# jkulhanek/viewformer

Measured on AMD Instinct MI355X. Metric: novel views/sec (encode->AR transformer->decode), 128px 6-ctx, higher is better.
Workload: dtype bf16

## Files before the change

__graft_entry__.py:

```python
import os
import sys

REPO = os.path.dirname(os.path.abspath(__file__))
if REPO not in sys.path:
    sys.path.insert(0, REPO)


def build() -> None:
    from viewformer_amd import build as vf_build
    lib = vf_build.build()
    assert os.path.exists(lib), lib
    var = vf_build.build_variant('trintrin')
    assert os.path.exists(var), var
    import viewformer_amd
    from viewformer_amd import _lib, vqgan, migt, evaluate
    _lib.load()
    import oracle.vqgan_oracle, oracle.migt_oracle, oracle.pipeline_oracle
    print('built', lib)


def smoke() -> None:
    import numpy as np
    import torch
    assert torch.cuda.is_available(), 'smoke() needs the MI355X'
    from viewformer_amd.config import VQGANConfig, MIGTConfig
    from viewformer_amd.weights import make_vqgan_weights, make_migt_weights, synthetic_scene_batch
    from viewformer_amd.vqgan import VQGAN
    from viewformer_amd.migt import MIGT
    from viewformer_amd.evaluate import generate_batch_predictions
    from oracle import pipeline_oracle as po

    dev = torch.device('cuda:0')
    vcfg = VQGANConfig(ch=32, ch_mult=[1, 2, 4], num_res_blocks=1, attn_resolutions=[16], image_size=32,
                       z_channels=32, embed_dim=32, n_embed=128)
    mcfg = MIGTConfig(n_embeddings=128, n_head=2, d_model=128, n_layer=2, token_image_size=8, sequence_size=3,
                      pose_multiplier=0.2)
    vsd = make_vqgan_weights(vcfg, seed=1, codebook_scale=0.05)
    msd = make_migt_weights(mcfg, seed=1, std=0.05)
    frames, cams = synthetic_scene_batch(2, 3, 32, seed=2)
    vq = VQGAN(vcfg, data_format='NHWC').load_state_dict(vsd).to(dev)
    tr = MIGT(mcfg).load_state_dict(msd).to(dev)
    got = generate_batch_predictions(tr, vq, frames, cams, return_codes=True)
    torch.cuda.synchronize()
    ref = po.generate_batch_predictions(msd, mcfg, vsd, vcfg, frames, cams, return_intermediates=True)
    assert torch.equal(got['codes'].cpu(), ref['codes']), 'context token indices differ from the oracle'
    err = (got['logits_last'].cpu() - ref['logits_last']).abs().max().item()
    assert err < 1e-3, err
    agree = (got['generated_codes'].cpu() == ref['generated_codes']).float().mean().item()
    assert agree > 0.95, agree
    print(f'smoke ok: context codes bit-exact, logit err {err:.2e}, generated-code agreement {agree:.3f}')


if __name__ == '__main__':
    build()
    if len(sys.argv) > 1 and sys.argv[1] == 'smoke':
        smoke()
```

viewformer_amd/build.py:

```python
import os
import subprocess
import sys

HERE = os.path.dirname(os.path.abspath(__file__))
CSRC = os.path.join(HERE, 'csrc')
LIB = os.path.join(HERE, 'libvf_hip.so')
ARCH = 'gfx950'
EXTRA_FLAGS = {'conv3_halo_x3h': ['-fno-slp-vectorize']}


def sources():
    return sorted(os.path.join(CSRC, f) for f in os.listdir(CSRC) if f.endswith('.hip'))


def _stale():
    if not os.path.exists(LIB):
        return True
    t = os.path.getmtime(LIB)
    deps = sources() + [os.path.join(CSRC, f) for f in os.listdir(CSRC) if f.endswith('.h')]
    deps.append(os.path.join(os.path.dirname(HERE), 'include', 'vf_hip.h'))
    return any(os.path.getmtime(d) > t for d in deps)


def build(force: bool = False, verbose: bool = False) -> str:
    if not force and not _stale():
        return LIB
    hipcc = os.environ.get('HIPCC', '/opt/rocm/bin/hipcc')
    objs = []
    procs = []
    os.makedirs(os.path.join(HERE, 'build'), exist_ok=True)
    stems = {os.path.basename(s)[:-4] for s in sources()}
    for f in os.listdir(os.path.join(HERE, 'build')):
        if f.endswith('.o') and f[:-2] not in stems:
            os.remove(os.path.join(HERE, 'build', f))
    for src in sources():
        obj = os.path.join(HERE, 'build', os.path.basename(src)[:-4] + '.o')
        cmd = [hipcc, f'--offload-arch={ARCH}', '-O3', '-std=c++17', '-fPIC', '-c', src, '-o', obj,
               '-Wall', '-Wno-unused-function'] + EXTRA_FLAGS.get(os.path.basename(src)[:-4], [])
        if verbose:
            cmd.append('-Rpass-analysis=kernel-resource-usage')
        procs.append((src, subprocess.Popen(cmd, stdout=subprocess.PIPE, stderr=subprocess.STDOUT, text=True)))
        objs.append(obj)
    failed = False
    for src, p in procs:
        out, _ = p.communicate()
        if p.returncode != 0 or verbose:
            sys.stderr.write(f'--- {os.path.basename(src)}\n{out}\n')
        failed |= p.returncode != 0
    if failed:
        raise RuntimeError('hipcc failed')
    cmd = [hipcc, f'--offload-arch={ARCH}', '-shared', '-fPIC', '-o', LIB] + objs
    subprocess.check_call(cmd)
    return LIB


VARIANTS = {
    'trintrin': (['-DVF_X_TRINTRIN'], ['attention_dma', 'attention_train_bf16', 'gemm_tn_bf16']),
}


def variant_path(name: str) -> str:
    return os.path.join(HERE, 'variants', f'libvf_{name}.so')


def build_variant(name: str, force: bool = False) -> str:
    flags, stems = VARIANTS[name]
    build()
    out = variant_path(name)
    srcs = [os.path.join(CSRC, st + '.hip') for st in stems]
    hdrs = [os.path.join(CSRC, f) for f in os.listdir(CSRC) if f.endswith('.h')]
    if not force and os.path.exists(out) and all(os.path.getmtime(d) <= os.path.getmtime(out) for d in srcs + hdrs + [LIB]):
        return out
    hipcc = os.environ.get('HIPCC', '/opt/rocm/bin/hipcc')
    os.makedirs(os.path.dirname(out), exist_ok=True)
    procs, vobjs = [], []
    for st, src in zip(stems, srcs):
        obj = os.path.join(HERE, 'variants', f'{st}.{name}.o')
        cmd = [hipcc, f'--offload-arch={ARCH}', '-O3', '-std=c++17', '-fPIC', '-w', '-c', src, '-o', obj] + EXTRA_FLAGS.get(st, []) + flags
        procs.append(subprocess.Popen(cmd))
        vobjs.append(obj)
    if any(p.wait() != 0 for p in procs):
        raise RuntimeError(f'hipcc failed on variant {name}')
    objs = [os.path.join(HERE, 'build', os.path.basename(s)[:-4] + '.o') for s in sources() if os.path.basename(s)[:-4] not in stems]
    subprocess.check_call([hipcc, f'--offload-arch={ARCH}', '-shared', '-fPIC', '-o', out] + objs + vobjs)
    return out


if __name__ == '__main__':
    print(build(force='--force' in sys.argv, verbose='-v' in sys.argv))
```

viewformer_amd/csrc/conv3_halo_bf16.hip:

```cpp
#include "halo_common.h"

namespace {

typedef __bf16 bf16x8 __attribute__((ext_vector_type(8)));
typedef __bf16 bf16x4 __attribute__((ext_vector_type(4)));

constexpr int CK = 32;
constexpr int P_LDB = 80;
constexpr int TH = 8, TW = 16;
constexpr int BN = 128;
constexpr int TAP_BYTES = CK * BN * 2;

template <bool UP2, bool PAIR = false>
struct Geo {
    static constexpr int PH = UP2 ? (TH / 2 + 2) : (TH + 2);
    static constexpr int PW = PAIR ? 20 : (UP2 ? (TW / 2 + 2) : (TW + 2));
    static constexpr int NPIX = PH * PW;
    static constexpr int SLOTS = (NPIX * 8 + 255) / 256;
    static constexpr int BUF = (NPIX + 1) * P_LDB;
};

__device__ __forceinline__ float fast_swish(float t) {
    return t * __builtin_amdgcn_rcpf(1.0f + __builtin_amdgcn_exp2f(-1.4426950408889634f * t));
}
// ... 95 lines not shown
    if (PAIR) { img = bid * 2; }
    else { tx = bid % tilesX; bid /= tilesX; ty = bid % tilesY; img = bid / tilesY; }
    const int n_img_total = p.M / (p.Hout * p.Wout);
    const int img1 = PAIR ? min(img + 1, n_img_total - 1) : img;
    const int pair_pix = (img1 - img) * p.Hin * p.Win;
    const int y0 = ty * TH, x0 = tx * TW;
    const int sy0 = UP2 ? (y0 / 2 - 1) : (y0 - 1);
    const int sx0 = UP2 ? (x0 / 2 - 1) : (x0 - 1);

    const float* __restrict__ X = p.x + (size_t)img * p.Hin * p.Win * p.Cin;
    const int nchunks = p.Cin / CK;
    const int last_stage = nchunks * 9 - 1;

    const int c4 = tid & 7;
    int s_off[G::SLOTS];
    bool s_ok[G::SLOTS];
    int s_sel[G::SLOTS];
    int s_lds[G::SLOTS];
#pragma unroll
    for (int q = 0; q < G::SLOTS; ++q) {
        const int pix = (tid >> 3) + 32 * q;
        const int pixc = pix < G::NPIX ? pix : G::NPIX;
        const int pr = pixc / G::PW, pc0 = pixc - pr * G::PW;
        const int sel = PAIR ? (pc0 >= 10) : 0;
        const int pc = pc0 - 10 * sel;
        s_sel[q] = sel;
        const int sy = sy0 + pr, sx = sx0 + pc;
        const bool ok = pix < G::NPIX && sy >= 0 && sy < p.Hin && sx >= 0 && sx < p.Win;
        s_ok[q] = ok;
        s_off[q] = ok ? (sel * pair_pix + sy * p.Win + sx) * p.Cin + c4 * 4 : c4 * 4;
        s_lds[q] = pixc * P_LDB + c4 * 8;
    }

    f32x4 preg[G::SLOTS];
    f32x4 pa, pb, pa1, pb1;
    const __amdgpu_buffer_rsrc_t x_rs = __builtin_amdgcn_make_buffer_rsrc(const_cast<float*>(X), 0, 0x7fffffff, 0x00020000);
    auto patch_load = [&](int chunk) {
#pragma unroll
        for (int q = 0; q < G::SLOTS; ++q)
            preg[q] = __builtin_bit_cast(f32x4, __builtin_amdgcn_raw_buffer_load_b128(x_rs, (unsigned)s_off[q] * 4u, (unsigned)(chunk * CK * 4), 0));
        if (PRO) {
            const f32x4 pmean = *reinterpret_cast<const f32x4*>(p.pro_mean + (size_t)img * p.Cin + chunk * CK + c4 * 4);
            const f32x4 pbeta = *reinterpret_cast<const f32x4*>(p.pro_beta + chunk * CK + c4 * 4);
            pa = *reinterpret_cast<const f32x4*>(p.pro_scale + (size_t)img * p.Cin + chunk * CK + c4 * 4);
#pragma unroll
            for (int e = 0; e < 4; ++e) pb[e] = __builtin_fmaf(-pmean[e], pa[e], pbeta[e]);
            if (PAIR) {
                const f32x4 pmean1 = *reinterpret_cast<const f32x4*>(p.pro_mean + (size_t)img1 * p.Cin + chunk * CK + c4 * 4);
                pa1 = *reinterpret_cast<const f32x4*>(p.pro_scale + (size_t)img1 * p.Cin + chunk * CK + c4 * 4);
#pragma unroll
                for (int e = 0; e < 4; ++e) pb1[e] = __builtin_fmaf(-pmean1[e], pa1[e], pbeta[e]);
            }
        }
    };
    auto patch_store_slot = [&](int buf, int q) {
        unsigned char* dst = smem_h + buf * G::BUF;
        bf16x4 o;
#pragma unroll
        for (int e = 0; e < 4; ++e) {
            float t = preg[q][e];
            if (PRO) {
                t = __builtin_fmaf(t, (PAIR && s_sel[q]) ? pa1[e] : pa[e], (PAIR && s_sel[q]) ? pb1[e] : pb[e]);
                if (SWISH) t = fast_swish(t);
            }
            o[e] = (__bf16)(s_ok[q] ? t : 0.f);
        }
        *reinterpret_cast<bf16x4*>(dst + s_lds[q]) = o;
    };

    const int trow = vf_perm_row(l31), tpx = vf_perm_px(l31);
    int a_base[MI], a_r[MI];
#pragma unroll
    for (int mi = 0; mi < MI; ++mi) {
        const int a0 = wave_m * 4 + mi * 2 + trow;
        a_r[mi] = a0;
        const int tcol = PAIR ? (tpx >> 3) * 10 + (tpx & 7) : tpx;
        a_base[mi] = (a0 * G::PW + tcol) * P_LDB + half * 16;
    }

    const unsigned char* __restrict__ Wb = reinterpret_cast<const unsigned char*>(p.w_packed) + (size_t)nblk * TAP_BYTES;
    const size_t tap_stride = (size_t)nb * TAP_BYTES;
    const int b_lane = (half * BN + wave_n * (32 * NJ) + l31) * 16;
    constexpr int BD = 2, RING = BD + 1;
    static_assert(9 % RING == 0, "ring indices must repeat per chunk");
    bf16x8 bring[RING][2 * NJ];
    bf16x8 aring[2][MI][2];
    const int last_g = nchunks * 9 - 1;
    const __amdgpu_buffer_rsrc_t w_rs = __builtin_amdgcn_make_buffer_rsrc(const_cast<unsigned char*>(Wb), 0, 0x7fffffff, 0x00020000);
    auto b_load = [&](bf16x8 (&dst)[2 * NJ], int g) {
        const unsigned soff = (unsigned)((size_t)min(g, last_g) * tap_stride);
#pragma unroll
        for (int ks = 0; ks < 2; ++ks)
#pragma unroll
            for (int j = 0; j < NJ; ++j)
                dst[ks * NJ + j] = __builtin_bit_cast(bf16x8, __builtin_amdgcn_raw_buffer_load_b128(w_rs, (unsigned)((ks * 2 * BN + j * 32) * 16 + b_lane), soff, 0));
    };
    auto a_load = [&](bf16x8 (&dst)[MI][2], const unsigned char* patch, int tap) {
        const int dy = tap / 3, dx = tap % 3;
#pragma unroll
        for (int mi = 0; mi < MI; ++mi) {
            int aoff;
            if (UP2) {
                const int pr = (a_r[mi] + dy + 1) >> 1, pc = (tpx + dx + 1) >> 1;
                aoff = (pr * G::PW + pc) * P_LDB + half * 16;
            } else {
                aoff = a_base[mi] + (dy * G::PW + dx) * P_LDB;
            }
#pragma unroll
            for (int ks = 0; ks < 2; ++ks) dst[mi][ks] = *reinterpret_cast<const bf16x8*>(patch + aoff + ks * 32);
        }
    };

    f32x16 acc[MI][NJ];
#pragma unroll
    for (int i = 0; i < MI; ++i)
#pragma unroll
        for (int j = 0; j < NJ; ++j)
#pragma unroll
            for (int r = 0; r < 16; ++r) acc[i][j][r] = 0.f;

    patch_load(0);
#pragma unroll
    for (int g = 0; g < BD; ++g) b_load(bring[g], g);
#pragma unroll
    for (int q = 0; q < G::SLOTS; ++q) patch_store_slot(0, q);
    __syncthreads();

    for (int chunk = 0; chunk < nchunks; ++chunk) {
        const unsigned char* patch = smem_h + (chunk & 1) * G::BUF;
        patch_load(min(chunk + 1, nchunks - 1));
        a_load(aring[0], patch, 0);
#pragma unroll
        for (int tap = 0; tap < 9; ++tap) {
            b_load(bring[(tap + BD) % RING], chunk * 9 + tap + BD);
            if (tap + 1 < 9) a_load(aring[(tap + 1) & 1], patch, tap + 1);
#pragma unroll
            for (int ks = 0; ks < 2; ++ks)
#pragma unroll
                for (int mi = 0; mi < MI; ++mi)
#pragma unroll
                    for (int j = 0; j < NJ; ++j)
                        acc[mi][j] = __builtin_amdgcn_mfma_f32_32x32x16_bf16(aring[tap & 1][mi][ks], bring[tap % RING][ks * NJ + j], acc[mi][j], 0, 0, 0);
            __builtin_amdgcn_sched_barrier(0);
            if (tap >= 1 && tap <= G::SLOTS) patch_store_slot((chunk + 1) & 1, tap - 1);
        }
        __syncthreads();
    }

    if constexpr (OUT16) halo_epilogue16<MI, NJ>(p, acc, img, y0, x0, (ty * tilesX + tx) * 2, nblk, wave_m, wave_n, half, l31);
    else vf_halo_epilogue_t<PAIR, MI, NJ>(p, acc, img, img1, y0, x0, PAIR ? 0 : (ty * tilesX + tx) * 2, nblk, wave_m, wave_n, half, l31);
}


template <bool UP2, bool PRO, bool SWISH>
__global__ __launch_bounds__(128, 2) void conv3_halo_bf16_w2_kernel(vf_igemm_args p) {
    using G = Geo<UP2, false>;
    constexpr int SLOTS = (G::NPIX + 31) / 32;
    constexpr int MI = 4, NJ = 2;
    extern __shared__ __attribute__((aligned(16))) unsigned char smem_h[];
    typedef unsigned u32x4 __attribute__((ext_vector_type(4)));

    const int tid = threadIdx.x;
    const int lane = tid & 63;
    const int wave_n = __builtin_amdgcn_readfirstlane(tid >> 6);
    const int half = lane >> 5, l31 = lane & 31;

    const int nb = p.Cout / BN;
    const int tilesX = p.Wout / TW, tilesY = p.Hout / TH;
    int bid = (int)vf_xcd_bid();
    const int nblk = bid % nb; bid /= nb;
    const int tx = bid % tilesX; bid /= tilesX;
    const int ty = bid % tilesY;
    const int img = bid / tilesY;
    const int y0 = ty * TH, x0 = tx * TW;
    const int sy0 = UP2 ? (y0 / 2 - 1) : (y0 - 1);
    const int sx0 = UP2 ? (x0 / 2 - 1) : (x0 - 1);
    const __bf16* __restrict__ X = reinterpret_cast<const __bf16*>(p.x) + (size_t)img * p.Hin * p.Win * p.Cin;
    const int nchunks = p.Cin / CK;

    const int c8 = tid & 3;
    int s_off[SLOTS], s_lds[SLOTS];
    unsigned ok_mask = 0;
#pragma unroll
    for (int q = 0; q < SLOTS; ++q) {
        const int pix = (tid >> 2) + 32 * q;
        const int pixc = pix < G::NPIX ? pix : G::NPIX;
        const int pr = pixc / G::PW, pc = pixc - pr * G::PW;
        const int sy = sy0 + pr, sx = sx0 + pc;
        const bool ok = pix < G::NPIX && sy >= 0 && sy < p.Hin && sx >= 0 && sx < p.Win;
        ok_mask |= (unsigned)ok << q;
        s_off[q] = (ok ? (sy * p.Win + sx) * p.Cin + c8 * 8 : c8 * 8) * 2;
        s_lds[q] = pixc * P_LDB + c8 * 16;
    }
    u32x4 preg[SLOTS];
    float pa[8], pb[8];
    const __amdgpu_buffer_rsrc_t x_rs = __builtin_amdgcn_make_buffer_rsrc(const_cast<__bf16*>(X), 0, 0x7fffffff, 0x00020000);
    auto patch_load = [&](int chunk) {
#pragma unroll
        for (int q = 0; q < SLOTS; ++q)
            preg[q] = __builtin_bit_cast(u32x4, __builtin_amdgcn_raw_buffer_load_b128(x_rs, (unsigned)s_off[q], (unsigned)(chunk * CK * 2), 0));
        if (PRO) {
#pragma unroll
            for (int h = 0; h < 2; ++h) {
                const int c = chunk * CK + c8 * 8 + h * 4;
                const f32x4 mu = *reinterpret_cast<const f32x4*>(p.pro_mean + (size_t)img * p.Cin + c);
                const f32x4 sc = *reinterpret_cast<const f32x4*>(p.pro_scale + (size_t)img * p.Cin + c);
                const f32x4 be = *reinterpret_cast<const f32x4*>(p.pro_beta + c);
#pragma unroll
                for (int e = 0; e < 4; ++e) { pa[h * 4 + e] = sc[e]; pb[h * 4 + e] = __builtin_fmaf(-mu[e], sc[e], be[e]); }
            }
        }
    };
    auto patch_store_slot = [&](int buf, int q) {
        unsigned char* dst = smem_h + buf * G::BUF;
        const bool ok = (ok_mask >> q) & 1u;
        bf16x8 o;
#pragma unroll
        for (int e = 0; e < 8; ++e) {
            const unsigned w = preg[q][e >> 1];
            float t = __builtin_bit_cast(float, (e & 1) ? (w & 0xffff0000u) : (w << 16));
            if (PRO) {
                t = __builtin_fmaf(t, pa[e], pb[e]);
                if (SWISH) t = fast_swish(t);
            }
            o[e] = (__bf16)t;
        }
        u32x4 ow = __builtin_bit_cast(u32x4, o);
#pragma unroll
        for (int e = 0; e < 4; ++e) ow[e] = ok ? ow[e] : 0u;
        *reinterpret_cast<u32x4*>(dst + s_lds[q]) = ow;
    };

    const int trow = vf_perm_row(l31), tpx = vf_perm_px(l31);
    int a_base[MI];
#pragma unroll
    for (int mi = 0; mi < MI; ++mi) a_base[mi] = ((mi * 2 + trow) * G::PW + tpx) * P_LDB + half * 16;

    const unsigned char* __restrict__ Wb = reinterpret_cast<const unsigned char*>(p.w_packed) + (size_t)nblk * TAP_BYTES;
    const size_t tap_stride = (size_t)nb * TAP_BYTES;
    const int b_lane = (half * BN + wave_n * (32 * NJ) + l31) * 16;
    constexpr int BD = 2, RB = BD + 1;
    static_assert(18 % RB == 0, "ring indices must repeat per chunk");
    bf16x8 bring[RB][NJ];
    bf16x8 aring[2][MI];
    const int last_g = nchunks * 9 - 1;
    const __amdgpu_buffer_rsrc_t w_rs = __builtin_amdgcn_make_buffer_rsrc(const_cast<unsigned char*>(Wb), 0, 0x7fffffff, 0x00020000);
    auto b_load = [&](bf16x8 (&dst)[NJ], int g2) {
        const unsigned soff = (unsigned)((size_t)min(g2 >> 1, last_g) * tap_stride);
        const int ks = g2 & 1;
#pragma unroll
        for (int j = 0; j < NJ; ++j)
            dst[j] = __builtin_bit_cast(bf16x8, __builtin_amdgcn_raw_buffer_load_b128(w_rs, (unsigned)((ks * 2 * BN + j * 32) * 16 + b_lane), soff, 0));
    };
    auto a_load = [&](bf16x8 (&dst)[MI], const unsigned char* patch, int s) {
        const int tap = s >> 1, ks = s & 1;
        const int dy = tap / 3, dx = tap % 3;
#pragma unroll
        for (int mi = 0; mi < MI; ++mi) {
            int aoff;
            if (UP2) {
                const int pr = (mi * 2 + trow + dy + 1) >> 1, pc = (tpx + dx + 1) >> 1;
                aoff = (pr * G::PW + pc) * P_LDB + half * 16;
            } else {
                aoff = a_base[mi] + (dy * G::PW + dx) * P_LDB;
            }
            dst[mi] = *reinterpret_cast<const bf16x8*>(patch + aoff + ks * 32);
        }
    };

    f32x16 acc[MI][NJ];
#pragma unroll
    for (int i = 0; i < MI; ++i)
#pragma unroll
        for (int j = 0; j < NJ; ++j)
#pragma unroll
            for (int r = 0; r < 16; ++r) acc[i][j][r] = 0.f;

    patch_load(0);
#pragma unroll
    for (int s = 0; s < BD; ++s) b_load(bring[s], s);
#pragma unroll
    for (int q = 0; q < SLOTS; ++q) patch_store_slot(0, q);
    __syncthreads();

    for (int chunk = 0; chunk < nchunks; ++chunk) {
        const unsigned char* patch = smem_h + (chunk & 1) * G::BUF;
        const bool more = chunk + 1 < nchunks;
        if (more) patch_load(chunk + 1);
        a_load(aring[0], patch, 0);
#pragma unroll
        for (int s = 0; s < 18; ++s) {
            b_load(bring[(s + BD) % RB], chunk * 18 + s + BD);
            if (s + 1 < 18) a_load(aring[(s + 1) & 1], patch, s + 1);
#pragma unroll
            for (int mi = 0; mi < MI; ++mi)
#pragma unroll
                for (int j = 0; j < NJ; ++j) acc[mi][j] = __builtin_amdgcn_mfma_f32_32x32x16_bf16(aring[s & 1][mi], bring[s % RB][j], acc[mi][j], 0, 0, 0);
            __builtin_amdgcn_sched_barrier(0);
            if ((s & 1) && (s >> 1) < SLOTS && more) patch_store_slot((chunk + 1) & 1, s >> 1);
        }
        __syncthreads();
    }
    halo_epilogue16<MI, NJ>(p, acc, img, y0, x0, (ty * tilesX + tx) * 2, nblk, 0, wave_n, half, l31);
}

__global__ void pack_conv_bf16_kernel(const float* __restrict__ w, __bf16* __restrict__ dst, int Cin, int Cout, int nb, int nchunks) {
    const long long total = (long long)nchunks * 9 * nb * CK * BN;
    for (long long idx = blockIdx.x * (long long)blockDim.x + threadIdx.x; idx < total; idx += (long long)gridDim.x * blockDim.x) {
        const int e = (int)(idx & 7);
        long long t = idx >> 3;
        const int nl = (int)(t % BN); t /= BN;
        const int half = (int)(t & 1);
        const int ks = (int)((t >> 1) & 1);
        t >>= 2;
        const int nblk = (int)(t % nb); t /= nb;
        const int tap = (int)(t % 9);
        const int chunk = (int)(t / 9);
        const int c = chunk * CK + ks * 16 + half * 8 + e;
        const int n = nblk * BN + nl;
        float v = 0.f;
        if (c < Cin && n < Cout) v = w[((size_t)n * Cin + c) * 9 + tap];
        dst[idx] = (__bf16)v;
    }
}

template <bool UP2, bool PRO, bool SWISH, bool PAIR, int IO16 = 0>
int launch_halo(const vf_igemm_args& a, hipStream_t stream) {
    using G = Geo<UP2, PAIR>;
    const size_t smem = (size_t)2 * G::BUF;
    const int n_img = a.M / (a.Hout * a.Wout);
    const long long blocks = PAIR ? (long long)((n_img + 1) / 2) * (a.Cout / BN)
                                  : (long long)n_img * (a.Hout / TH) * (a.Wout / TW) * (a.Cout / BN);
    hipLaunchKernelGGL((conv3_halo_bf16_kernel<UP2, PRO, SWISH, PAIR, IO16>), dim3((unsigned)blocks), dim3(256), smem, stream, a);
    return vf_last_status();
}

template <bool UP2, bool PRO, bool SWISH>
int launch_halo_w2(const vf_igemm_args& a, hipStream_t stream) {
    using G = Geo<UP2, false>;
    const int n_img = a.M / (a.Hout * a.Wout);
    const long long blocks = (long long)n_img * (a.Hout / TH) * (a.Wout / TW) * (a.Cout / BN);
    hipLaunchKernelGGL((conv3_halo_bf16_w2_kernel<UP2, PRO, SWISH>), dim3((unsigned)blocks), dim3(128), (size_t)2 * G::BUF, stream, a);
    return vf_last_status();
}

template <bool UP2, bool PAIR, int IO16 = 0>
int dispatch_pro(const vf_igemm_args& a, hipStream_t s) {
    if (!a.pro_mean) return launch_halo<UP2, false, false, PAIR, IO16>(a, s);
    return a.pro_swish ? launch_halo<UP2, true, true, PAIR, IO16>(a, s) : launch_halo<UP2, true, false, PAIR, IO16>(a, s);
}
template <bool UP2>
int dispatch_io(const vf_igemm_args& a, hipStream_t s) {
    switch (a.reserved0 & 3) {
        case 0: return dispatch_pro<UP2, false, 0>(a, s);
        case 2: return dispatch_pro<UP2, false, 2>(a, s);
        case 3:
            if (a.Cin & 7) return VF_ERR_UNSUPPORTED;
            if (!a.pro_mean) return launch_halo_w2<UP2, false, false>(a, s);
            return a.pro_swish ? launch_halo_w2<UP2, true, true>(a, s) : launch_halo_w2<UP2, true, false>(a, s);
        default: return VF_ERR_UNSUPPORTED;
    }
}

}

extern "C" {

size_t vf_conv3_bf16_packed_elems(int Cin, int Cout) {
    if (Cin <= 0 || Cout <= 0) return 0;
    return (size_t)((Cin + CK - 1) / CK) * 9 * ((Cout + BN - 1) / BN) * CK * BN;
}

int vf_conv3_bf16_pack(const float* w_oihw, void* dst, int Cin, int Cout, void* stream) {
    if (!w_oihw || !dst || Cin <= 0 || Cout <= 0) return VF_ERR_BAD_ARG;
    const int nb = (Cout + BN - 1) / BN, nchunks = (Cin + CK - 1) / CK;
    const long long total = (long long)nchunks * 9 * nb * CK * BN;
    const int blocks = (int)((total + 255) / 256 > 4096 ? 4096 : (total + 255) / 256);
    hipLaunchKernelGGL(pack_conv_bf16_kernel, dim3(blocks), dim3(256), 0, (hipStream_t)stream, w_oihw, (__bf16*)dst, Cin, Cout, nb,
                       nchunks);
    return vf_last_status();
}

int vf_conv3_halo_bf16(const vf_igemm_args* args, void* stream) {
    if (!args) return VF_ERR_BAD_ARG;
    const vf_igemm_args& a = *args;
    if (!a.x || !a.w_packed || !a.out || a.M <= 0) return VF_ERR_BAD_ARG;
    if (a.drop_rate != 0.f || a.out_aux) return VF_ERR_UNSUPPORTED;
    if (a.mode != VF_MODE_CONV3_S1 && a.mode != VF_MODE_CONV3_UP2) return VF_ERR_UNSUPPORTED;
    const bool pair = a.mode == VF_MODE_CONV3_S1 && a.Hout == 8 && a.Wout == 8;
    if (a.Cout % BN != 0 || a.Cin % CK != 0 || (!pair && (a.Hout % TH != 0 || a.Wout % TW != 0))) return VF_ERR_UNSUPPORTED;
    if (a.Hin <= 0 || a.Win <= 0 || a.M % (a.Hout * a.Wout) != 0) return VF_ERR_BAD_ARG;
    if (a.mode == VF_MODE_CONV3_S1 && (a.Hout != a.Hin || a.Wout != a.Win)) return VF_ERR_BAD_ARG;
    if (a.mode == VF_MODE_CONV3_UP2 && (a.Hout != a.Hin * 2 || a.Wout != a.Win * 2)) return VF_ERR_BAD_ARG;
    if (a.batch > 1 || a.epilogue != VF_EPI_NONE || a.ldc < a.Cout || (a.res && a.ldr < a.Cout)) return VF_ERR_BAD_ARG;
    if ((a.pro_mean || a.pro_scale || a.pro_beta) && !(a.pro_mean && a.pro_scale && a.pro_beta)) return VF_ERR_BAD_ARG;
    if ((long long)a.Hin * a.Win * a.Cin >= (1ll << 31)) return VF_ERR_UNSUPPORTED;
    if (int st = vf_halo_gn_check(a)) return st;
    hipStream_t s = (hipStream_t)stream;
    if (a.reserved0 & ~3) return VF_ERR_BAD_ARG;
    if (a.reserved0 && (pair || (a.ldc & 1) || (a.res && (a.ldr & 1)) || (a.Cin & 3))) return VF_ERR_UNSUPPORTED;
    if (pair) return dispatch_pro<false, true>(a, s);
    return (a.mode == VF_MODE_CONV3_UP2) ? dispatch_io<true>(a, s) : dispatch_io<false>(a, s);
}

}
```

viewformer_amd/csrc/vf_common.h:

```cpp
#pragma once
#include <hip/hip_runtime.h>
#include <stdint.h>

typedef float f32x4 __attribute__((ext_vector_type(4)));
typedef float f32x16 __attribute__((ext_vector_type(16)));

#define VF_OK 0
#define VF_ERR_BAD_ARG (-1)
#define VF_ERR_UNSUPPORTED (-2)

#define VF_WAVE 64

static inline int vf_last_status() {
    hipError_t e = hipGetLastError();
    return e == hipSuccess ? VF_OK : (int)e;
}

static inline bool vf_attr_needed(unsigned long long* mask) {
    int d = 0;
    (void)hipGetDevice(&d);
    return !((__atomic_load_n(mask, __ATOMIC_RELAXED) >> (d & 63)) & 1ull);
}
static inline void vf_attr_done(unsigned long long* mask) {
    int d = 0;
    (void)hipGetDevice(&d);
    __atomic_fetch_or(mask, 1ull << (d & 63), __ATOMIC_RELAXED);
}

__device__ __forceinline__ float vf_swish(float v) {
    return v / (1.0f + expf(-v));
}

__device__ __forceinline__ float vf_swish_1ulp(float v) {
    const float LH = -1.4426950408889634f, LL = -1.9259629911266175e-8f;
    float th = v * LH;
    const float tl = __builtin_fmaf(v, LH, -th) + v * LL;
    th = fminf(th, 126.0f);
    const float e0 = __builtin_amdgcn_exp2f(th);
    const float d = 1.0f + __builtin_fmaf(e0 * tl, 0.6931471805599453f, e0);
    float r = __builtin_amdgcn_rcpf(d);
    r = __builtin_fmaf(__builtin_fmaf(-d, r, 1.0f), r, r);
    return v * r;
}

__device__ __forceinline__ float vf_exp_neg(float d) {
    const float LH = 1.4426950408889634f, LL = 1.9259629911266175e-8f;
    const float th = __fmul_rn(d, LH);
    const float tl = __builtin_fmaf(d, LH, -th) + d * LL;
    const float e0 = __builtin_amdgcn_exp2f(th);
    return __builtin_fmaf(e0 * tl, 0.6931471805599453f, e0);
}

__device__ __forceinline__ float vf_gelu_erf(float v) {
    return 0.5f * v * (1.0f + erff(v * 0.70710678118654752440f));
}

__device__ __forceinline__ float vf_gelu_grad(float x) {
    const float cdf = __fmul_rn(0.5f, __fadd_rn(1.0f, erff(__fmul_rn(x, 0.70710678118654752440f))));
    const float pdf = __fmul_rn(0.39894228040143267794f, expf(__fmul_rn(-0.5f, __fmul_rn(x, x))));
    return __fmaf_rn(x, pdf, cdf);
}

__device__ __forceinline__ float vf_gelu_grad_fast(float x) {
    const float z = __fmul_rn(fabsf(x), 0.70710678118654752440f);
    const float t = __builtin_amdgcn_rcpf(__fmaf_rn(0.3275911f, z, 1.0f));
    float p = __fmaf_rn(1.061405429f, t, -1.453152027f);
    p = __fmaf_rn(p, t, 1.421413741f);
    p = __fmaf_rn(p, t, -0.284496736f);
    p = __fmaf_rn(p, t, 0.254829592f);
    const float e = __builtin_amdgcn_exp2f(__fmul_rn(-1.4426950408889634f, __fmul_rn(z, z)));
    const float erf_abs = __fmaf_rn(-__fmul_rn(p, t), e, 1.0f);
    const float cdf = __fmul_rn(0.5f, __fadd_rn(1.0f, copysignf(erf_abs, x)));
    return __fmaf_rn(x, __fmul_rn(0.39894228040143267794f, e), cdf);
}

__device__ __forceinline__ float vf_gelu_erf_fast(float v) {
    const float z = fabsf(v) * 0.70710678118654752440f;
    float t = __builtin_amdgcn_rcpf(__builtin_fmaf(0.3275911f, z, 1.0f));
    float p = __builtin_fmaf(1.061405429f, t, -1.453152027f);
    p = __builtin_fmaf(p, t, 1.421413741f);
    p = __builtin_fmaf(p, t, -0.284496736f);
    p = __builtin_fmaf(p, t, 0.254829592f);
    const float e = __builtin_amdgcn_exp2f(-1.4426950408889634f * z * z);
    const float erf_abs = __builtin_fmaf(-p * t, e, 1.0f);
    return 0.5f * v * (1.0f + copysignf(erf_abs, v));
}

__device__ __forceinline__ void vf_gelu_and_grad_fast(float v, float& f, float& g) {
    const float z = fabsf(v) * 0.70710678118654752440f;
    float t = __builtin_amdgcn_rcpf(__builtin_fmaf(0.3275911f, z, 1.0f));
    float p = __builtin_fmaf(1.061405429f, t, -1.453152027f);
    p = __builtin_fmaf(p, t, 1.421413741f);
    p = __builtin_fmaf(p, t, -0.284496736f);
    p = __builtin_fmaf(p, t, 0.254829592f);
    const float e = __builtin_amdgcn_exp2f(-1.4426950408889634f * z * z);
    const float erf_abs = __builtin_fmaf(-p * t, e, 1.0f);
    const float one_plus = 1.0f + copysignf(erf_abs, v);
    f = 0.5f * v * one_plus;
    g = __builtin_fmaf(v, 0.39894228040143267794f * e, 0.5f * one_plus);
}

__device__ __forceinline__ int vf_lane_xor1(int v) { return __builtin_amdgcn_mov_dpp(v, 0xB1, 0xF, 0xF, true); }
__device__ __forceinline__ unsigned vf_lane_xor1(unsigned v) { return (unsigned)__builtin_amdgcn_mov_dpp((int)v, 0xB1, 0xF, 0xF, true); }
__device__ __forceinline__ float vf_lane_xor1(float v) { return __int_as_float(__builtin_amdgcn_mov_dpp(__float_as_int(v), 0xB1, 0xF, 0xF, true)); }

__device__ __forceinline__ float vf_wave_sum(float v) {
#pragma unroll
    for (int o = 32; o > 0; o >>= 1) v += __shfl_xor(v, o, 64);
    return v;
}

__device__ __forceinline__ float vf_wave_sum_dpp(float v) {
#define VF_DPP_ADD(ctrl, rmask) v += __int_as_float(__builtin_amdgcn_update_dpp(0, __float_as_int(v), ctrl, rmask, 0xF, false))
    VF_DPP_ADD(0x111, 0xF);
    VF_DPP_ADD(0x112, 0xF);
    VF_DPP_ADD(0x114, 0xF);
    VF_DPP_ADD(0x118, 0xF);
    VF_DPP_ADD(0x142, 0xA);
    VF_DPP_ADD(0x143, 0xC);
#undef VF_DPP_ADD
    return __int_as_float(__builtin_amdgcn_readlane(__float_as_int(v), 63));
}

__device__ __forceinline__ float vf_wave_max(float v) {
#pragma unroll
    for (int o = 32; o > 0; o >>= 1) v = fmaxf(v, __shfl_xor(v, o, 64));
    return v;
}

__device__ __forceinline__ void vf_block_max_atomic(float m, unsigned* out) {
    __shared__ float vf_bm_red[4];
    m = vf_wave_max(m);
    if ((threadIdx.x & 63) == 0) vf_bm_red[threadIdx.x >> 6] = m;
    __syncthreads();
    if (threadIdx.x == 0) atomicMax(out, __float_as_uint(fmaxf(fmaxf(vf_bm_red[0], vf_bm_red[1]), fmaxf(vf_bm_red[2], vf_bm_red[3]))));
}

__host__ __device__ __forceinline__ uint32_t vf_dropout_hash(uint32_t seed, uint32_t site, uint64_t idx) {
    uint32_t h = seed ^ (site * 0x9E3779B9u);
    h ^= (uint32_t)idx;
    h *= 0x85EBCA6Bu;
    h ^= h >> 13;
    h += (uint32_t)(idx >> 32) * 0xC2B2AE35u + 0x27D4EB2Fu;
    h ^= h >> 16;
    h *= 0x165667B1u;
    h ^= h >> 15;
    h *= 0xD3A2646Cu;
    h ^= h >> 16;
    return h;
}
__host__ __device__ __forceinline__ uint32_t vf_lowbias32(uint32_t x) {
    x ^= x >> 16;
    x *= 0x7FEB352Du;
    x ^= x >> 15;
    x *= 0x846CA68Bu;
    x ^= x >> 16;
    return x;
}
__host__ __device__ __forceinline__ uint32_t vf_dropout_key(uint32_t seed, uint32_t site, uint32_t hi) { return vf_dropout_hash(seed, site, (uint64_t)hi); }
__host__ __device__ __forceinline__ uint32_t vf_dropout_word(uint32_t key, uint32_t lo) { return vf_lowbias32(lo ^ key); }
__host__ __device__ __forceinline__ bool vf_dropout_keep(uint32_t word, int j, uint32_t thresh) {
    const uint32_t s = 8u * ((uint32_t)j & 3u);
    return ((word << s) | (word >> ((32u - s) & 31u))) >= thresh;
}
__device__ __forceinline__ uint32_t vf_dropout_rotr(int j) { return (32u - 8u * ((uint32_t)j & 3u)) & 31u; }
__device__ __forceinline__ bool vf_dropout_keep_rotr(uint32_t word, uint32_t rr, uint32_t thresh) { return __builtin_amdgcn_alignbit(word, word, rr) >= thresh; }
__host__ __device__ __forceinline__ bool vf_dropout_keep_elem(uint32_t seed, uint32_t site, uint64_t m, uint32_t n, uint32_t N, uint32_t thresh) {
    const uint64_t g = (m >> 2) * (uint64_t)N + n;
    return vf_dropout_keep(vf_dropout_word(vf_dropout_key(seed, site, (uint32_t)(g >> 32)), (uint32_t)g), (int)(m & 3), thresh);
}
__host__ __device__ __forceinline__ uint32_t vf_dropout_thresh(float rate) { return (uint32_t)((double)rate * 4294967296.0); }

__device__ __forceinline__ unsigned vf_xcd_bid() {
    const unsigned n = gridDim.x, b = blockIdx.x;
    const unsigned q = n >> 3, r = n & 7u, x = b & 7u, i = b >> 3;
    return x * q + (x < r ? x : r) + i;
}

__device__ __forceinline__ float vf_vq_sq4(const f32x4 v) {
    return __builtin_fmaf(v[0], v[0], v[1] * v[1]) + __builtin_fmaf(v[2], v[2], v[3] * v[3]);
}

extern "C" int vf_register_build_flag(const char* name);
#define VF_REG_FLAG(m) namespace { const int vf_flagreg_##m = vf_register_build_flag(#m); }
#ifdef VF_X_TRINTRIN
VF_REG_FLAG(VF_X_TRINTRIN)
#endif

int vf_pack_b_impl(const float* src, float* dst, int K, int N, int taps, long long sk, long long sn, long long st,
                   int BN, int batch, long long src_bstride, hipStream_t stream);

struct vf_attn_order { unsigned char blk[64]; };
static inline bool vf_attn_visible(int qv, int kv, int twin) {
    if (twin <= -2) {
        const int Sv = -twin, qs = qv / Sv, qi = qv - qs * Sv, ks = kv / Sv, ki = kv - ks * Sv;
        return qs == 0 ? (ks == 0 && ki <= qi) : ((ks == 0 && ki < qi) || kv == qv);
    }
    const int Vc = twin >= 0 ? twin : 0x3fffffff;
    return kv == qv || (kv < Vc ? kv : Vc) < (qv < Vc ? qv : Vc);
}
static inline vf_attn_order vf_attn_block_order(int nviews, int vpb, int nblocks, int twin, bool by_key) {
    vf_attn_order o;
    int w[64];
    if (nblocks > 64) nblocks = 64;
    for (int b = 0; b < 64; ++b) o.blk[b] = (unsigned char)b;
    for (int b = 0; b < nblocks; ++b) {
        int cnt = 0;
        for (int t = 0; t < nviews; ++t) {
            bool any = false;
            for (int v = b * vpb; v < (b + 1) * vpb && v < nviews && !any; ++v) any = by_key ? vf_attn_visible(t, v, twin) : vf_attn_visible(v, t, twin);
            cnt += any;
        }
        w[b] = cnt;
    }
    for (int i = 1; i < nblocks; ++i) {
        const unsigned char bi = o.blk[i];
        int j = i - 1;
        while (j >= 0 && w[o.blk[j]] < w[bi]) { o.blk[j + 1] = o.blk[j]; --j; }
        o.blk[j + 1] = bi;
    }
    return o;
}

struct vf_attn_groups { unsigned char view[64][4]; int n; };
static inline vf_attn_groups vf_attn_query_groups(int nviews, int twin) {
    vf_attn_groups g;
    for (int i = 0; i < 64; ++i) for (int j = 0; j < 4; ++j) g.view[i][j] = 0xFF;
    g.n = 0;
    unsigned char list[256];
    int nl = 0;
    const int Sv = twin <= -2 ? -twin : 0;
    if (Sv > 0 && nviews % Sv == 0 && nviews / Sv >= 2 && nviews <= 255) {
        const int NS = nviews / Sv;
        for (int v = 0; v < Sv; ++v) list[nl++] = (unsigned char)v;
        const int pad = (4 - Sv % 4) % 4;
        int taken = 0;
        unsigned char br[256];
        int nb = 0;
        for (int i = Sv - 1; i >= 0; --i)
            for (int s_ = 1; s_ < NS; ++s_) br[nb++] = (unsigned char)(s_ * Sv + i);
        for (; taken < pad && taken < nb; ++taken) list[nl++] = br[taken];
        while (nl % 4) list[nl++] = 0xFF;
        for (int i = taken; i < nb; ++i) list[nl++] = br[i];
    } else {
        for (int v = 0; v < nviews && v < 256; ++v) list[nl++] = (unsigned char)v;
    }
    while (nl % 4) list[nl++] = 0xFF;
    g.n = nl / 4 > 64 ? 64 : nl / 4;
    int w[64];
    for (int b = 0; b < g.n; ++b) {
        int cnt = 0;
        for (int t = 0; t < nviews; ++t) {
            bool any = false;
            for (int j = 0; j < 4 && !any; ++j) { const int v = list[4 * b + j]; any = v != 0xFF && vf_attn_visible(v, t, twin); }
            cnt += any;
        }
        w[b] = cnt;
    }
    int ord[64];
    for (int b = 0; b < g.n; ++b) ord[b] = b;
    for (int i = 1; i < g.n; ++i) {
        const int bi = ord[i];
        int j = i - 1;
        while (j >= 0 && w[ord[j]] < w[bi]) { ord[j + 1] = ord[j]; --j; }
        ord[j + 1] = bi;
    }
    for (int b = 0; b < g.n; ++b) for (int j = 0; j < 4; ++j) g.view[b][j] = list[4 * ord[b] + j];
    return g;
}

typedef __bf16 vf_bf16x8 __attribute__((ext_vector_type(8)));
typedef short vf_s16x4 __attribute__((ext_vector_type(4)));
__device__ __forceinline__ unsigned vf_lds_addr(const void* p) {
    return (unsigned)(size_t)(__attribute__((address_space(3))) const void*)p;
}
__device__ __forceinline__ vf_bf16x8 vf_tr_join(vf_s16x4 lo, vf_s16x4 hi) {
    return __builtin_bit_cast(vf_bf16x8, __builtin_shufflevector(lo, hi, 0, 1, 2, 3, 4, 5, 6, 7));
}
__device__ __forceinline__ void vf_tr_frag2_wait(vf_bf16x8& a, vf_bf16x8& b, unsigned addr, int offA, int offB, int gap) {
    vf_s16x4 a0, a1, b0, b1;
    asm volatile("ds_read_b64_tr_b16 %0, %4 offset:%5\n\tds_read_b64_tr_b16 %1, %4 offset:%6\n\tds_read_b64_tr_b16 %2, %4 offset:%7\n\t"
                 "ds_read_b64_tr_b16 %3, %4 offset:%8\n\ts_waitcnt lgkmcnt(0)"
                 : "=&v"(a0), "=&v"(a1), "=&v"(b0), "=&v"(b1) : "v"(addr), "i"(offA), "i"(offA + gap), "i"(offB), "i"(offB + gap) : "memory");
    a = vf_tr_join(a0, a1);
    b = vf_tr_join(b0, b1);
}
```

Measured before the change: 1156.

## Add 16x16x32 bf16 MFMA halo conv kernel with LDS-DMA staging for stride-1 convs

Adds a 256-thread 3x3 stride-1 conv kernel that uses 16x16x32 bf16 MFMA instructions. The next channel chunk's input patch is loaded with buffer-load-to-LDS DMA, then converted and stored into the alternate buffer, interleaved across taps. It also keeps register rings for A and B operands to overlap loads with compute. By default it replaces the existing path for eligible stride-1 convs, and a build variant flag turns it off for comparison. The cost is higher LDS and register use and a more complex epilogue for fused residual and GroupNorm stats.

Measured after the change: 1159, median of 6. No clear change (+0.3%).

```diff
diff --git a/__graft_entry__.py b/__graft_entry__.py
--- a/__graft_entry__.py
+++ b/__graft_entry__.py
@@ -11,6 +11,8 @@
     lib = vf_build.build()
     assert os.path.exists(lib), lib
     var = vf_build.build_variant('trintrin')
+    assert os.path.exists(var), var
+    var = vf_build.build_variant('convbf16_mfma32')
     assert os.path.exists(var), var
     import viewformer_amd
     from viewformer_amd import _lib, vqgan, migt, evaluate
diff --git a/viewformer_amd/build.py b/viewformer_amd/build.py
--- a/viewformer_amd/build.py
+++ b/viewformer_amd/build.py
@@ -56,6 +56,7 @@
 
 VARIANTS = {
     'trintrin': (['-DVF_X_TRINTRIN'], ['attention_dma', 'attention_train_bf16', 'gemm_tn_bf16']),
+    'convbf16_mfma32': (['-DVF_X_CONV_BF16_MFMA32'], ['conv3_halo_bf16']),
 }
 
 
diff --git a/viewformer_amd/csrc/conv3_halo_bf16.hip b/viewformer_amd/csrc/conv3_halo_bf16.hip
--- a/viewformer_amd/csrc/conv3_halo_bf16.hip
+++ b/viewformer_amd/csrc/conv3_halo_bf16.hip
@@ -421,6 +421,294 @@
         __syncthreads();
     }
     halo_epilogue16<MI, NJ>(p, acc, img, y0, x0, (ty * tilesX + tx) * 2, nblk, 0, wave_n, half, l31);
+}
+
+typedef float f32x4v __attribute__((ext_vector_type(4)));
+constexpr int K32_AR = 4;
+
+template <int IO16>
+constexpr int k32_slots() { return (IO16 & 1) ? 3 : 6; }
+
+template <bool PRO, bool SWISH, int IO16>
+__global__ __launch_bounds__(256, (IO16 & 1) ? 3 : 2) void conv3_halo_bf16_k32_kernel(vf_igemm_args p) {
+    static_assert(IO16 == 0 || IO16 == 2 || IO16 == 3, "fp32 in / fp32 out, fp32 in / bf16 out, bf16 in / bf16 out");
+    constexpr bool IN16 = (IO16 & 1) != 0, OUT16 = (IO16 & 2) != 0;
+    using G = Geo<false, false>;
+    constexpr int RT = 8, CT = 2;
+    constexpr int SLOTS = k32_slots<IO16>();
+    constexpr int TPP = IN16 ? 4 : 8;
+    constexpr int PPS = 256 / TPP;
+    constexpr int ESZ = IN16 ? 2 : 4;
+    constexpr int AR = K32_AR;
+    static_assert(72 % AR == 0, "ring indices must repeat per chunk");
+    static_assert(3 + SLOTS <= 9, "one staging slot per tap from tap 3 on");
+    extern __shared__ __attribute__((aligned(16))) unsigned char smem_h[];
+    typedef unsigned u32x4 __attribute__((ext_vector_type(4)));
+
+    const int tid = threadIdx.x;
+    const int lane = tid & 63;
+    const int wave = __builtin_amdgcn_readfirstlane(tid >> 6);
+    const int lm = lane & 15, lg = lane >> 4;
+
+    const int nb = p.Cout / BN;
+    const int tilesX = p.Wout / TW, tilesY = p.Hout / TH;
+    int bid = (int)vf_xcd_bid();
+    const int nblk = bid % nb; bid /= nb;
+    const int tx = bid % tilesX; bid /= tilesX;
+    const int ty = bid % tilesY;
+    const int img = bid / tilesY;
+    const int y0 = ty * TH, x0 = tx * TW;
+    const int sy0 = y0 - 1, sx0 = x0 - 1;
+    const unsigned char* __restrict__ X = reinterpret_cast<const unsigned char*>(p.x) + (size_t)img * p.Hin * p.Win * p.Cin * ESZ;
+    const int nchunks = p.Cin / CK;
+
+    const int cq = tid & (TPP - 1);
+    const int cqs = IN16 ? ((cq & 1) * 2 + (cq >> 1)) * 16
+                         : (((cq >> 1) & 1) * 2 + (cq >> 2)) * 16 + (cq & 1) * 8;
+    const int lds0 = (tid / TPP) * P_LDB + cqs;
+    int pix0 = tid / TPP;
+    auto slot_src = [&](int q, bool& ok) {
+        const int pix = pix0 + PPS * q;
+        const int pixc = min(pix, (int)G::NPIX);
+        const int pr = (pixc * 3641) >> 16, pc = pixc - pr * G::PW;
+        const int sy = sy0 + pr, sx = sx0 + pc;
+        ok = (pix < G::NPIX) & ((unsigned)sy < (unsigned)p.Hin) & ((unsigned)sx < (unsigned)p.Win);
+        const int off = (sy * p.Win + sx) * p.Cin;
+        return (ok ? off : 0) + cq * (IN16 ? 8 : 4);
+    };
+    unsigned ok_mask = 0;
+    int lds_last = 0;
+#pragma unroll
+    for (int q = 0; q < SLOTS; ++q) {
+        bool ok;
+        (void)slot_src(q, ok);
+        ok_mask |= (unsigned)ok << q;
+        if (q == SLOTS - 1) lds_last = min(pix0 + PPS * q, (int)G::NPIX) * P_LDB + cqs;
+    }
+    unsigned char* __restrict__ raw_l = smem_h + 2 * G::BUF;
+    float* __restrict__ pro_l = reinterpret_cast<float*>(raw_l + SLOTS * 4096);
+    const __amdgpu_buffer_rsrc_t x_rs = __builtin_amdgcn_make_buffer_rsrc(const_cast<unsigned char*>(X), 0, 0x7fffffff, 0x00020000);
+    if (PRO) {
+        for (int i = tid; i < p.Cin; i += 256) {
+            const float sc = p.pro_scale[(size_t)img * p.Cin + i];
+            pro_l[i] = sc;
+            pro_l[p.Cin + i] = __builtin_fmaf(-p.pro_mean[(size_t)img * p.Cin + i], sc, p.pro_beta[i]);
+        }
+    }
+    int pro_chunk = 0;
+    auto patch_load = [&](int chunk) {
+        asm volatile("" : "+v"(pix0));
+#pragma unroll
+        for (int q = 0; q < SLOTS; ++q) {
+            bool ok;
+            const int off = slot_src(q, ok);
+            __builtin_amdgcn_raw_ptr_buffer_load_lds(x_rs, (__attribute__((address_space(3))) void*)(raw_l + q * 4096 + wave * 1024), 16,
+                                                     (unsigned)off * (unsigned)ESZ, (unsigned)(chunk * CK * ESZ), 0, 0);
+        }
+        pro_chunk = chunk;
+    };
+    auto patch_store_slot = [&](int buf, int q) {
+        unsigned char* dst = smem_h + buf * G::BUF + (q == SLOTS - 1 ? lds_last : lds0 + q * PPS * P_LDB);
+        const bool ok = (ok_mask >> q) & 1u;
+        constexpr int NE = IN16 ? 8 : 4;
+        float t[NE];
+        const f32x4 rawf = *reinterpret_cast<const f32x4*>(raw_l + q * 4096 + tid * 16);
+        const u32x4 raw = __builtin_bit_cast(u32x4, rawf);
+#pragma unroll
+        for (int e = 0; e < NE; ++e) {
+            if constexpr (IN16) t[e] = __builtin_bit_cast(float, (e & 1) ? (raw[e >> 1] & 0xffff0000u) : (raw[e >> 1] << 16));
+            else t[e] = rawf[e];
+        }
+        if (PRO) {
+            const float* pl = pro_l + pro_chunk * CK + cq * NE;
+#pragma unroll
+            for (int h = 0; h < NE / 4; ++h) {
+                const f32x4 a = *reinterpret_cast<const f32x4*>(pl + h * 4);
+                const f32x4 b = *reinterpret_cast<const f32x4*>(pl + p.Cin + h * 4);
+#pragma unroll
+                for (int e = 0; e < 4; ++e) {
+                    float v = __builtin_fmaf(t[h * 4 + e], a[e], b[e]);
+                    if (SWISH) v = fast_swish(v);
+                    t[h * 4 + e] = v;
+                }
+            }
+        }
+        if (IN16) {
+            bf16x8 o;
+#pragma unroll
+            for (int e = 0; e < 8; ++e) o[e] = (__bf16)t[e];
+            u32x4 ow = __builtin_bit_cast(u32x4, o);
+#pragma unroll
+            for (int e = 0; e < 4; ++e) ow[e] = ok ? ow[e] : 0u;
+            *reinterpret_cast<u32x4*>(dst) = ow;
+        } else {
+            bf16x4 o;
+#pragma unroll
+            for (int e = 0; e < 4; ++e) o[e] = (__bf16)(ok ? t[e] : 0.f);
+            *reinterpret_cast<bf16x4*>(dst) = o;
+        }
+    };
+
+    const int lpix = lm < 4 ? 2 * lm : lm < 12 ? 2 * lm - 7 : 2 * lm - 16;
+    const int a_lane = lpix * P_LDB + (((lg & 1) * 2) + (lg >> 1)) * 16;
+    const unsigned char* __restrict__ Wb = reinterpret_cast<const unsigned char*>(p.w_packed) + (size_t)nblk * TAP_BYTES;
+    const size_t tap_stride = (size_t)nb * TAP_BYTES;
+    const int b_lane = lg * (BN * 16) + (wave * 32 + lm) * 16;
+    const int last_tap = nchunks * 9 - 1;
+    const __amdgpu_buffer_rsrc_t w_rs = __builtin_amdgcn_make_buffer_rsrc(const_cast<unsigned char*>(Wb), 0, 0x7fffffff, 0x00020000);
+    bf16x8 bring[3][CT];
+    bf16x8 aring[AR];
+    auto b_load = [&](bf16x8 (&dst)[CT], int gtap) {
+        const unsigned soff = (unsigned)((size_t)min(gtap, last_tap) * tap_stride);
+#pragma unroll
+        for (int ct = 0; ct < CT; ++ct)
+            dst[ct] = __builtin_bit_cast(bf16x8, __builtin_amdgcn_raw_buffer_load_b128(w_rs, (unsigned)(b_lane + ct * 256), soff, 0));
+    };
+    auto a_load = [&](bf16x8& dst, const unsigned char* patch, int step) {
+        const int tap = step >> 3, rt = step & 7;
+        dst = *reinterpret_cast<const bf16x8*>(patch + a_lane + ((rt + tap / 3) * G::PW + tap % 3) * P_LDB);
+    };
+
+    f32x4v acc[RT][CT];
+#pragma unroll
+    for (int i = 0; i < RT; ++i)
+#pragma unroll
+        for (int j = 0; j < CT; ++j)
+#pragma unroll
+            for (int r = 0; r < 4; ++r) acc[i][j][r] = 0.f;
+
+    patch_load(0);
+    b_load(bring[0], 0);
+    b_load(bring[1], 1);
+    asm volatile("s_waitcnt vmcnt(0)" ::: "memory");
+    if (PRO) __syncthreads();
+#pragma unroll
+    for (int q = 0; q < SLOTS; ++q) patch_store_slot(0, q);
+    __syncthreads();
+
+    auto chunk_body = [&](int chunk, auto parity) {
+        constexpr int P0 = decltype(parity)::value;
+        const unsigned char* patch = smem_h + P0 * G::BUF;
+        const bool more = chunk + 1 < nchunks;
+        b_load(bring[2], chunk * 9 + 2);
+        patch_load(min(chunk + 1, nchunks - 1));
+#pragma unroll
+        for (int i = 0; i < AR - 1; ++i) a_load(aring[i], patch, i);
+#pragma unroll
+        for (int t = 0; t < 9; ++t) {
+            if (t > 0) b_load(bring[(t + 2) % 3], chunk * 9 + t + 2);
+            const bf16x8 (&B)[CT] = bring[t % 3];
+#pragma unroll
+            for (int rt = 0; rt < RT; ++rt) {
+                const int step = t * 8 + rt;
+                if (step + AR - 1 < 72) a_load(aring[(step + AR - 1) % AR], patch, step + AR - 1);
+                const bf16x8 a = aring[step % AR];
+                acc[rt][0] = __builtin_amdgcn_mfma_f32_16x16x32_bf16(a, B[0], acc[rt][0], 0, 0, 0);
+                acc[rt][1] = __builtin_amdgcn_mfma_f32_16x16x32_bf16(a, B[1], acc[rt][1], 0, 0, 0);
+                __builtin_amdgcn_sched_barrier(0);
+            }
+            if (t >= 3 && t < 3 + SLOTS && more) {
+                if (t == 3) {
+                    if (SLOTS == 3) asm volatile("s_waitcnt vmcnt(8)" ::: "memory");
+                    else asm volatile("s_waitcnt vmcnt(11)" ::: "memory");
+                }
+                patch_store_slot((P0 + 1) & 1, t - 3);
+            }
+        }
+        __syncthreads();
+    };
+    for (int chunk = 0; chunk < nchunks; chunk += 2) {
+        chunk_body(chunk, std::integral_constant<int, 0>{});
+        chunk_body(chunk + 1, std::integral_constant<int, 1>{});
+    }
+
+    constexpr int OSZ = OUT16 ? 2 : 4;
+    unsigned char* out_b = reinterpret_cast<unsigned char*>(p.out) + (size_t)img * p.Hout * p.Wout * p.ldc * OSZ;
+    const unsigned char* res_b = p.res ? reinterpret_cast<const unsigned char*>(p.res) + (size_t)img * p.Hout * p.Wout * p.ldr * OSZ : out_b;
+    const __amdgpu_buffer_rsrc_t o_rs = __builtin_amdgcn_make_buffer_rsrc(out_b, 0, 0x7fffffff, 0x00020000);
+    const __amdgpu_buffer_rsrc_t r_rs = __builtin_amdgcn_make_buffer_rsrc(const_cast<unsigned char*>(res_b), 0, 0x7fffffff, 0x00020000);
+    const bool Res = p.res != nullptr;
+    const bool stats = p.gn_part != nullptr;
+    const int cg = p.Cout >> 5;
+    const int tile_slot = (ty * tilesX + tx) * 2;
+    const int pbase = lg == 0 ? 0 : lg == 1 ? 1 : lg == 2 ? 9 : 8;
+    const int odd = lm & 1;
+    auto spix = [&](int rt, int r) { return (y0 + rt) * p.Wout + x0 + 2 * r; };
+    constexpr int RW = OUT16 ? 2 : 4;
+    unsigned rr[CT][RT][RW];
+    if (Res) {
+#pragma unroll
+        for (int ct = 0; ct < CT; ++ct) {
+            const int n = nblk * BN + wave * 32 + ct * 16 + lm;
+            const unsigned rv = OUT16 ? (unsigned)((pbase + 2 * odd) * p.ldr + n - odd) * 2u : (unsigned)(pbase * p.ldr + n) * 4u;
+#pragma unroll
+            for (int rt = 0; rt < RT; ++rt)
+#pragma unroll
+                for (int k = 0; k < RW; ++k)
+                    rr[ct][rt][k] = __builtin_amdgcn_raw_buffer_load_b32(r_rs, rv, (unsigned)(spix(rt, OUT16 ? 2 * k : k) * p.ldr) * (unsigned)OSZ, 0);
+        }
+    }
+#pragma unroll
+    for (int ct = 0; ct < CT; ++ct) {
+        const int n = nblk * BN + wave * 32 + ct * 16 + lm;
+        const float bias = p.bias ? p.bias[n] : 0.f;
+        const unsigned ov = OUT16 ? (unsigned)((pbase + 2 * odd) * p.ldc + n - odd) * 2u : (unsigned)(pbase * p.ldc + n) * 4u;
+#pragma unroll
+        for (int sl = 0; sl < 2; ++sl) {
+            float s32 = 0.f, q32 = 0.f;
+#pragma unroll
+            for (int k4 = 0; k4 < 4; ++k4) {
+                const int rt = sl * 4 + k4;
+                float v[4];
+#pragma unroll
+                for (int r = 0; r < 4; ++r) v[r] = acc[rt][ct][r] + bias;
+                if (Res) {
+                    if (OUT16) {
+#pragma unroll
+                        for (int k = 0; k < 2; ++k) {
+                            const unsigned mine = rr[ct][rt][k];
+                            const unsigned give = odd ? (mine << 16) : (mine & 0xffff0000u);
+                            const unsigned got = vf_lane_xor1(give);
+                            v[2 * k] += __builtin_bit_cast(float, odd ? got : (mine << 16));
+                            v[2 * k + 1] += __builtin_bit_cast(float, odd ? (mine & 0xffff0000u) : got);
+                        }
+                    } else {
+#pragma unroll
+                        for (int r = 0; r < 4; ++r) v[r] += __builtin_bit_cast(float, rr[ct][rt][r]);
+                    }
+                }
+#pragma unroll
+                for (int r = 0; r < 4; ++r) { s32 += v[r]; q32 = __builtin_fmaf(v[r], v[r], q32); }
+                if (OUT16) {
+                    typedef __bf16 bf16x2_t __attribute__((ext_vector_type(2)));
+#pragma unroll
+                    for (int k = 0; k < 2; ++k) {
+                        const float give = odd ? v[2 * k] : v[2 * k + 1];
+                        const float got = vf_lane_xor1(give);
+                        bf16x2_t h;
+                        h[0] = (__bf16)(odd ? got : v[2 * k]);
+                        h[1] = (__bf16)(odd ? v[2 * k + 1] : got);
+                        __builtin_amdgcn_raw_buffer_store_b32(__builtin_bit_cast(unsigned, h), o_rs, ov, (unsigned)(spix(rt, 2 * k) * p.ldc) * 2u, 0);
+                    }
+                } else {
+#pragma unroll
+                    for (int r = 0; r < 4; ++r)
+                        __builtin_amdgcn_raw_buffer_store_b32(__builtin_bit_cast(unsigned, v[r]), o_rs, ov, (unsigned)(spix(rt, r) * p.ldc) * 4u, 0);
+                }
+            }
+            if (stats) {
+                vf_gn_acc_t s = (vf_gn_acc_t)s32, q = (vf_gn_acc_t)q32;
+                for (int o = 1; o < cg; o <<= 1) { s += __shfl_xor(s, o, 64); q += __shfl_xor(q, o, 64); }
+                s += __shfl_xor(s, 16, 64); q += __shfl_xor(q, 16, 64);
+                s += __shfl_xor(s, 32, 64); q += __shfl_xor(q, 32, 64);
+                if (lg == 0 && (lm & (cg - 1)) == 0) {
+                    float* dst = p.gn_part + ((((size_t)img * p.gn_slots) + tile_slot + sl) * 32 + n / cg) * 2;
+                    dst[0] = (float)s;
+                    dst[1] = (float)q;
+                }
+            }
+        }
+    }
 }
 
 __global__ void pack_conv_bf16_kernel(const float* __restrict__ w, __bf16* __restrict__ dst, int Cin, int Cout, int nb, int nchunks) {
@@ -461,6 +749,37 @@
     const long long blocks = (long long)n_img * (a.Hout / TH) * (a.Wout / TW) * (a.Cout / BN);
     hipLaunchKernelGGL((conv3_halo_bf16_w2_kernel<UP2, PRO, SWISH>), dim3((unsigned)blocks), dim3(128), (size_t)2 * G::BUF, stream, a);
     return vf_last_status();
+}
+
+static inline size_t k32_lds_bytes(bool in16, int pro_cin) {
+    return (size_t)2 * Geo<false, false>::BUF + (size_t)(in16 ? k32_slots<3>() : k32_slots<0>()) * 4096 + (size_t)2 * pro_cin * 4;
+}
+
+static inline bool k32_takes(const vf_igemm_args& a) {
+#ifdef VF_X_CONV_BF16_MFMA32
+    return false;
+#else
+    if (a.mode != VF_MODE_CONV3_S1 || a.Hout % TH != 0 || a.Wout % TW != 0) return false;
+    if ((a.Cin / CK) % 2 != 0) return false;
+    if (a.gn_part && a.Cout / 32 > 16) return false;
+    if (k32_lds_bytes(false, a.pro_mean ? a.Cin : 0) > 64 * 1024) return false;
+    const long long in_b = (long long)a.Hin * a.Win * a.Cin * 4, out_b = (long long)a.Hout * a.Wout * (a.ldc > a.ldr ? a.ldc : a.ldr) * 4;
+    return in_b < (1ll << 31) && out_b < (1ll << 31);
+#endif
+}
+
+template <bool PRO, bool SWISH, int IO16>
+int launch_k32(const vf_igemm_args& a, hipStream_t stream) {
+    const int n_img = a.M / (a.Hout * a.Wout);
+    const long long blocks = (long long)n_img * (a.Hout / TH) * (a.Wout / TW) * (a.Cout / BN);
+    hipLaunchKernelGGL((conv3_halo_bf16_k32_kernel<PRO, SWISH, IO16>), dim3((unsigned)blocks), dim3(256), k32_lds_bytes(IO16 & 1, PRO ? a.Cin : 0),
+                       stream, a);
+    return vf_last_status();
+}
+template <int IO16>
+int dispatch_k32(const vf_igemm_args& a, hipStream_t s) {
+    if (!a.pro_mean) return launch_k32<false, false, IO16>(a, s);
+    return a.pro_swish ? launch_k32<true, true, IO16>(a, s) : launch_k32<true, false, IO16>(a, s);
 }
 
 template <bool UP2, bool PAIR, int IO16 = 0>
@@ -519,6 +838,14 @@
     if (a.reserved0 & ~3) return VF_ERR_BAD_ARG;
     if (a.reserved0 && (pair || (a.ldc & 1) || (a.res && (a.ldr & 1)) || (a.Cin & 3))) return VF_ERR_UNSUPPORTED;
     if (pair) return dispatch_pro<false, true>(a, s);
+    if (k32_takes(a)) {
+        switch (a.reserved0 & 3) {
+            case 0: return dispatch_k32<0>(a, s);
+            case 2: return dispatch_k32<2>(a, s);
+            case 3: return dispatch_k32<3>(a, s);
+            default: return VF_ERR_UNSUPPORTED;
+        }
+    }
     return (a.mode == VF_MODE_CONV3_UP2) ? dispatch_io<true>(a, s) : dispatch_io<false>(a, s);
 }
 
diff --git a/viewformer_amd/csrc/vf_common.h b/viewformer_amd/csrc/vf_common.h
--- a/viewformer_amd/csrc/vf_common.h
+++ b/viewformer_amd/csrc/vf_common.h
@@ -185,6 +185,9 @@
 #define VF_REG_FLAG(m) namespace { const int vf_flagreg_##m = vf_register_build_flag(#m); }
 #ifdef VF_X_TRINTRIN
 VF_REG_FLAG(VF_X_TRINTRIN)
+#endif
+#ifdef VF_X_CONV_BF16_MFMA32
+VF_REG_FLAG(VF_X_CONV_BF16_MFMA32)
 #endif
 
 int vf_pack_b_impl(const float* src, float* dst, int K, int N, int taps, long long sk, long long sn, long long st,
```
